# aiforvision/OCTA-autosegmentation

Hardware: AMD Instinct MI355X
Metric: synthetic OCTA samples/sec (graph + 304x304 image + 1216x1216 label triples) (higher is better)
Workload: dtype f64

## Files before the change

### include/octa_hip.h

```cpp
#ifndef OCTA_HIP_H
#define OCTA_HIP_H

#include <stddef.h>
#include <stdint.h>

#ifdef __cplusplus
extern "C" {
#endif

typedef struct octa_ctx octa_ctx;


int octa_abi_version(void);

const char *octa_last_error(void);

int octa_ctx_create(int device, octa_ctx **out);
void octa_ctx_destroy(octa_ctx *ctx);

size_t octa_ctx_scratch_bytes(const octa_ctx *ctx);

int octa_rasterize_2d(octa_ctx *ctx, int B, const double *d_edges, const int64_t *h_edge_off,
                      const uint8_t *d_keep, int no_pixels_x, int no_pixels_y, int mip_axis,
                      double min_radius, double max_radius, uint8_t *d_out, void *stream);
// ... 227 lines not shown

int octa_sim_run_states(octa_sim *sim, const double *h_faz_radius, const double *h_stumps, const uint32_t *h_np_states,
                        const uint32_t *h_py_states, octa_bif_fn bif, void *user, void *stream);
int octa_sim_np_state(octa_sim *sim, int sample, uint32_t *h_state625);

int octa_sim_edge_offsets(octa_sim *sim, int64_t *h_edge_off, int64_t *h_n_art);

int octa_sim_export_edges(octa_sim *sim, double *h_edges);

int octa_sim_export_edges_device(octa_sim *sim, double *d_edges, void *stream);

int octa_sim_trace(octa_sim *sim, int32_t *h_trace);

int octa_sim_stats(octa_sim *sim, int64_t *h_stats);

int octa_sim_spans(octa_sim *sim, int64_t *h_spans);

int octa_sim_timing(octa_sim *sim, double *h_out8);

int octa_sim_service_stats(octa_sim *sim, double *h_out5);

int octa_sim_geometry(int num_cus, int *h_out4);

int octa_sim_is_large(const octa_sim *sim);

int octa_sim_fields(octa_sim *sim, int sample, double *h_oxy, int64_t cap_oxy, int64_t *n_oxy, double *h_co2,
                    int64_t cap_co2, int64_t *n_co2);

int octa_sim_kat_kd_order(octa_ctx *ctx, const double *h_pts, int64_t n, const uint8_t *h_need, int32_t *h_indices);

// ... 5 lines not shown
```

### octa_autosegmentation_amd/_native.py

```python
import contextlib
import ctypes
import os
import random as _random
import threading

import numpy as np

HERE = os.path.dirname(os.path.abspath(__file__))
LIB_PATH = os.environ.get("OCTA_HIP_LIB") or os.path.join(HERE, "liboctahip.so")

_lib = None
_ctxs = {}
_lock = threading.Lock()

c_void_p, c_int, c_double, c_size_t = ctypes.c_void_p, ctypes.c_int, ctypes.c_double, ctypes.c_size_t

SIGNATURES = {
    "octa_abi_version": (c_int, []),
    "octa_last_error": (ctypes.c_char_p, []),
    "octa_ctx_create": (c_int, [c_int, ctypes.POINTER(c_void_p)]),
    "octa_ctx_destroy": (None, [c_void_p]),
    "octa_ctx_scratch_bytes": (c_size_t, [c_void_p]),
    "octa_rasterize_2d": (c_int, [c_void_p, c_int, c_void_p, c_void_p, c_void_p, c_int, c_int, c_int, c_double,
                                  c_double, c_void_p, c_void_p]),
# ... 28 lines not shown
    "octa_sim_destroy": (None, [c_void_p]),
    "octa_sim_run": (c_int, [c_void_p, c_void_p, c_void_p, c_void_p, c_void_p, c_void_p]),
    "octa_sim_run_states": (c_int, [c_void_p, c_void_p, c_void_p, c_void_p, c_void_p, c_void_p, c_void_p, c_void_p]),
    "octa_sim_np_state": (c_int, [c_void_p, c_int, c_void_p]),
    "octa_thinconv_expand": (c_int, [c_void_p, c_void_p, c_void_p, c_void_p, c_void_p, c_int, c_int, c_int, c_int, c_int, c_int, c_int, ctypes.c_float, c_void_p]),
    "octa_thinconv_squeeze": (c_int, [c_void_p, c_void_p, c_void_p, c_void_p, c_void_p, c_int, c_int, c_int, c_int, c_int, c_int, c_int, c_void_p]),
    "octa_lrelu_bwd_bf16": (c_int, [c_void_p, c_void_p, c_void_p, c_void_p, ctypes.c_int64, ctypes.c_float, c_void_p]),
    "octa_thinconv_wgrad_scratch_floats": (ctypes.c_longlong, [c_int, c_int, c_int, c_int]),
    "octa_thinconv_wgrad": (c_int, [c_void_p, c_void_p, c_void_p, c_void_p, c_void_p, c_void_p, c_int, c_int, c_int, c_int, c_int, c_int, c_int, c_int, c_int, c_void_p]),
    "octa_sim_spans": (c_int, [c_void_p, c_void_p]),
    "octa_sim_edge_offsets": (c_int, [c_void_p, c_void_p, c_void_p]),
    "octa_sim_export_edges": (c_int, [c_void_p, c_void_p]),
    "octa_sim_export_edges_device": (c_int, [c_void_p, c_void_p, c_void_p]),
    "octa_sim_trace": (c_int, [c_void_p, c_void_p]),
    "octa_sim_stats": (c_int, [c_void_p, c_void_p]),
    "octa_sim_timing": (c_int, [c_void_p, c_void_p]),
    "octa_sim_service_stats": (c_int, [c_void_p, c_void_p]),
    "octa_sim_geometry": (c_int, [c_int, c_void_p]),
    "octa_sim_is_large": (c_int, [c_void_p]),
    "octa_conv2d_f32_nchw": (c_int, [c_void_p, c_void_p, c_void_p, c_void_p, c_void_p] + [c_int] * 14 + [c_void_p]),
    "octa_convtranspose2x2_f32_nchw": (c_int, [c_void_p, c_void_p, c_void_p, c_void_p, c_int, c_int, c_int, c_int, c_int, c_void_p]),
    "octa_conv2d_f32_dgrad_nchw": (c_int, [c_void_p, c_void_p, c_void_p, c_void_p] + [c_int] * 11 + [c_void_p]),
    "octa_conv2d_f32_wgrad_workspace": (c_int, [c_int] * 10 + [ctypes.POINTER(c_size_t)]),
    "octa_conv2d_f32_wgrad_nchw": (c_int, [c_void_p, c_void_p, c_void_p, c_void_p, c_void_p, c_void_p, c_size_t] + [c_int] * 10 + [c_void_p]),
    "octa_sim_fields": (c_int, [c_void_p, c_int, c_void_p, ctypes.c_int64, c_void_p, c_void_p, ctypes.c_int64, c_void_p]),
    "octa_instnorm_lrelu_nhwc_fwd": (c_int, [c_void_p, c_void_p, c_void_p, c_void_p, c_void_p, c_void_p, c_void_p, c_int, c_int, ctypes.c_int64, ctypes.c_float, ctypes.c_float, c_void_p]),
    "octa_instnorm_lrelu_nhwc_bwd": (c_int, [c_void_p, c_void_p, c_void_p, c_void_p, c_void_p, c_void_p, c_void_p, c_void_p, c_void_p, c_void_p, c_int, c_int, ctypes.c_int64, ctypes.c_float, c_void_p]),
    "octa_head1_nhwc_fwd": (c_int, [c_void_p, c_void_p, c_void_p, ctypes.c_float, ctypes.c_int64, c_int, c_void_p, c_void_p]),
    "octa_head1_nhwc_fwd_b": (c_int, [c_void_p, c_void_p, c_void_p, c_void_p, ctypes.c_int64, c_int, c_void_p, c_void_p]),
    "octa_pack_conv_weights": (c_int, [c_void_p, c_void_p, c_int, c_void_p, c_void_p]),
# ... 153 lines not shown
```

### octa_autosegmentation_amd/csrc/sim.hip

```cpp

#include <chrono>
#include <vector>

#include "common.h"
#include "sim_host.h"
#include <thread>
#include <atomic>
#include <cstdlib>
#include <cstring>

using namespace OCTA_SIMK;

#if OCTA_SIM_LARGE
#define OCTA_SIM_T octa_simL_impl
#define OCTA_SIM_FN(name) octa_simL_##name
#else
#define OCTA_SIM_T octa_simS_impl
#define OCTA_SIM_FN(name) octa_simS_##name
#endif
#define octa_sim_create OCTA_SIM_FN(create)
#define octa_sim_destroy OCTA_SIM_FN(destroy)
#define octa_sim_run OCTA_SIM_FN(run)
#define octa_sim_run_states OCTA_SIM_FN(run_states)
#define octa_sim_np_state OCTA_SIM_FN(np_state)
#define octa_sim_edge_offsets OCTA_SIM_FN(edge_offsets)
#define octa_sim_export_edges OCTA_SIM_FN(export_edges)
#define octa_sim_export_edges_device OCTA_SIM_FN(export_edges_device)
#define octa_sim_trace OCTA_SIM_FN(trace)
#define octa_sim_stats OCTA_SIM_FN(stats)
#define octa_sim_fields OCTA_SIM_FN(fields)
#define octa_sim_service_stats OCTA_SIM_FN(service_stats)
#define octa_sim_geometry OCTA_SIM_FN(geometry)
#define octa_sim_spans OCTA_SIM_FN(spans)
#define octa_sim_timing OCTA_SIM_FN(timing)
#define octa_sim_kat_kd_order OCTA_SIM_FN(kat_kd_order)
struct OCTA_SIM_T;
extern "C" void octa_sim_destroy(OCTA_SIM_T *S);
extern "C" long long octa_sim_next_ticket(void);
extern "C" int *octa_sim_launch_flag(int device);

namespace {

constexpr int SIM_THREADS = SIM_THREADS_PER_WG;
constexpr int SIM_WG_PER_CU = 2;
// ... 1217 lines not shown

extern "C" int octa_sim_stats(OCTA_SIM_T *S, int64_t *h_stats) {
    if (!S || !S->ran || !h_stats) { octa::set_error("octa_sim_stats: run the simulation first"); return -2; }
    for (int s = 0; s < S->B; s++) {
        const SampleScalars &sc = S->h_sc[s];
        int64_t *o = h_stats + 32 * s;
        o[0] = sc.err; o[1] = sc.py_pos; o[2] = sc.murray_steps; o[3] = sc.n_bif; o[4] = sc.respec;
        o[5] = sc.n_nodes[0]; o[6] = sc.n_nodes[1];
        memcpy(&o[7], &sc.faz_radius, 8);
        for (int k = 0; k < 16; k++) o[8 + k] = sc.prof[k];
        for (int k = 0; k < 8; k++) o[24 + k] = sc.kdprof[k];
    }
    return 0;
}

extern "C" int octa_sim_fields(OCTA_SIM_T *S, int sample, double *h_oxy, int64_t cap_oxy, int64_t *n_oxy, double *h_co2,
                               int64_t cap_co2, int64_t *n_co2) {
    if (!S || !S->ran || sample < 0 || sample >= S->B) { octa::set_error("octa_sim_fields: bad arguments"); return -2; }
    OCTA_HIP_CHECK(hipSetDevice(S->ctx->device));
    const SampleScalars &sc = S->h_sc[sample];
    if (n_oxy) *n_oxy = sc.n_oxy;
    if (n_co2) *n_co2 = sc.n_co2;
    if (h_oxy) {
        int64_t n = sc.n_oxy < cap_oxy ? sc.n_oxy : cap_oxy;
        OCTA_HIP_CHECK(hipMemcpy(h_oxy, S->P.oxy + (size_t)sample * OCAP * 3, sizeof(double) * 3 * n, hipMemcpyDeviceToHost));
    }
    if (h_co2) {
        int64_t n = sc.n_co2 < cap_co2 ? sc.n_co2 : cap_co2;
        OCTA_HIP_CHECK(hipMemcpy(h_co2, S->P.co2 + (size_t)sample * CCAP * 3, sizeof(double) * 3 * n, hipMemcpyDeviceToHost));
    }
// ... 69 lines not shown
```

### octa_autosegmentation_amd/csrc/sim_api.cpp

```cpp
#include <cstdlib>
#include <cstring>
#include <new>

#include "common.h"

extern "C" {
struct octa_simS_impl;
struct octa_simL_impl;
#define OCTA_DECL(SFX, T)                                                                                                                       \
    int octa_sim##SFX##_create(octa_ctx *, const octa_sim_config *, int, T **);                                                                 \
    void octa_sim##SFX##_destroy(T *);                                                                                                          \
    int octa_sim##SFX##_run(T *, const uint32_t *, const uint64_t *, octa_bif_fn, void *, void *);                                              \
    int octa_sim##SFX##_run_states(T *, const double *, const double *, const uint32_t *, const uint32_t *, octa_bif_fn, void *, void *);       \
    int octa_sim##SFX##_np_state(T *, int, uint32_t *);                                                                                         \
    int octa_sim##SFX##_edge_offsets(T *, int64_t *, int64_t *);                                                                                \
    int octa_sim##SFX##_export_edges(T *, double *);                                                                                            \
    int octa_sim##SFX##_export_edges_device(T *, double *, void *);                                                                             \
    int octa_sim##SFX##_trace(T *, int32_t *);                                                                                                  \
    int octa_sim##SFX##_stats(T *, int64_t *);                                                                                                  \
    int octa_sim##SFX##_spans(T *, int64_t *);                                                                                                  \
    int octa_sim##SFX##_timing(T *, double *);                                                                                                  \
    int octa_sim##SFX##_service_stats(T *, double *);                                                                                           \
    int octa_sim##SFX##_geometry(int, int *);                                                                                                   \
    int octa_sim##SFX##_fields(T *, int, double *, int64_t, int64_t *, double *, int64_t, int64_t *);
OCTA_DECL(S, octa_simS_impl)
OCTA_DECL(L, octa_simL_impl)
#undef OCTA_DECL
int octa_simS_kat_kd_order(octa_ctx *, const double *, int64_t, const uint8_t *, int32_t *);
}

#include <atomic>
#include <mutex>
static std::atomic<long long> g_sim_launches{0};
extern "C" long long octa_sim_next_ticket(void) { return g_sim_launches.fetch_add(1, std::memory_order_acq_rel) + 1; }
// ... 56 lines not shown
#define NEED(sim, what) if (!(sim)) { octa::set_error(what ": null simulator"); return -2; }
extern "C" int octa_sim_run(octa_sim *sim, const uint32_t *a, const uint64_t *b, octa_bif_fn f, void *u, void *st) {
    NEED(sim, "octa_sim_run") return FWD(octa_simS_run(sim->s, a, b, f, u, st), octa_simL_run(sim->l, a, b, f, u, st));
}
extern "C" int octa_sim_run_states(octa_sim *sim, const double *fz, const double *stp, const uint32_t *a, const uint32_t *b, octa_bif_fn f, void *u, void *st) {
    NEED(sim, "octa_sim_run_states") return FWD(octa_simS_run_states(sim->s, fz, stp, a, b, f, u, st), octa_simL_run_states(sim->l, fz, stp, a, b, f, u, st));
}
extern "C" int octa_sim_np_state(octa_sim *sim, int k, uint32_t *o) { NEED(sim, "octa_sim_np_state") return FWD(octa_simS_np_state(sim->s, k, o), octa_simL_np_state(sim->l, k, o)); }
extern "C" int octa_sim_edge_offsets(octa_sim *sim, int64_t *a, int64_t *b) { NEED(sim, "octa_sim_edge_offsets") return FWD(octa_simS_edge_offsets(sim->s, a, b), octa_simL_edge_offsets(sim->l, a, b)); }
extern "C" int octa_sim_export_edges(octa_sim *sim, double *e) { NEED(sim, "octa_sim_export_edges") return FWD(octa_simS_export_edges(sim->s, e), octa_simL_export_edges(sim->l, e)); }
extern "C" int octa_sim_export_edges_device(octa_sim *sim, double *e, void *st) {
    NEED(sim, "octa_sim_export_edges_device") return FWD(octa_simS_export_edges_device(sim->s, e, st), octa_simL_export_edges_device(sim->l, e, st));
}
extern "C" int octa_sim_trace(octa_sim *sim, int32_t *t) { NEED(sim, "octa_sim_trace") return FWD(octa_simS_trace(sim->s, t), octa_simL_trace(sim->l, t)); }
extern "C" int octa_sim_stats(octa_sim *sim, int64_t *t) { NEED(sim, "octa_sim_stats") return FWD(octa_simS_stats(sim->s, t), octa_simL_stats(sim->l, t)); }
extern "C" int octa_sim_spans(octa_sim *sim, int64_t *t) { NEED(sim, "octa_sim_spans") return FWD(octa_simS_spans(sim->s, t), octa_simL_spans(sim->l, t)); }
extern "C" int octa_sim_timing(octa_sim *sim, double *t) { NEED(sim, "octa_sim_timing") return FWD(octa_simS_timing(sim->s, t), octa_simL_timing(sim->l, t)); }
extern "C" int octa_sim_service_stats(octa_sim *sim, double *t) { NEED(sim, "octa_sim_service_stats") return FWD(octa_simS_service_stats(sim->s, t), octa_simL_service_stats(sim->l, t)); }
extern "C" int octa_sim_fields(octa_sim *sim, int k, double *o, int64_t co, int64_t *no, double *c, int64_t cc, int64_t *nc) {
    NEED(sim, "octa_sim_fields") return FWD(octa_simS_fields(sim->s, k, o, co, no, c, cc, nc), octa_simL_fields(sim->l, k, o, co, no, c, cc, nc));
}
extern "C" int octa_sim_geometry(int num_cus, int *h_out4) { return octa_simS_geometry(num_cus, h_out4); }
extern "C" int octa_sim_kat_kd_order(octa_ctx *ctx, const double *p, int64_t n, const uint8_t *need, int32_t *o) { return octa_simS_kat_kd_order(ctx, p, n, need, o); }
extern "C" int octa_sim_is_large(const octa_sim *sim) { return sim && sim->large ? 1 : 0; }
```

### octa_autosegmentation_amd/csrc/sim_core.h

```cpp
#pragma once
#include <cmath>
#include <cstdint>
#include <cstring>
#include <algorithm>
#include "gpow.h"
#include "glibc_trig.h"

#ifndef OCTA_SIM_LARGE
#define OCTA_SIM_LARGE 0
#endif
#if OCTA_SIM_LARGE
#define OCTA_SIMK octa_simk_large
#else
#define OCTA_SIMK octa_simk
#endif
namespace OCTA_SIMK {

#if OCTA_SIM_LARGE
typedef unsigned int idx_t;
typedef unsigned long long kdw_t;
constexpr int IDX_BITS = 18;
constexpr int GROUP_BITS = 17;
constexpr int NCAP = 1 << 17;
constexpr int OCAP = 1 << 18;
// ... 89 lines not shown
    int py_pos, py_cap;
    int err;
    int new_begin[2], new_end[2];
    int n_groups[2];
    int n_sorted[2];
    int n_grow[2];
    int pass_tag[2];
    int pass_counter;
    long murray_steps;
    long flush_rounds;
    long murray_deferred;
    long n_bif;
    long respec;
    long prof[16];
    long kdprof[8];
    int resume_it, resume_stage;
    int parked, finished;
    long t_begin, t_end;
    int fl_pending[2];
};

struct SimArrays {
    double *npos[2];
    double *nrad[2];
    double *nkap[2];
    int *npar[2], *nch0[2], *nch1[2];
    unsigned char *nnch[2], *nact[2];
    OCTA_HD double *npos_of(int f) const { return f ? npos[1] : npos[0]; }
    OCTA_HD double *nrad_of(int f) const { return f ? nrad[1] : nrad[0]; }
    OCTA_HD double *nkap_of(int f) const { return f ? nkap[1] : nkap[0]; }
// ... 382 lines not shown
            if (s.key[e] < 0) {
                s.fill++; s.used++;
                s.key[e] = key; s.hash[e] = hash;
                if (!OCTA_UNLIKELY(!((long)s.fill * 5 < (long)s.mask * 3))) return;
                pyset_resize(s, s.used > 50000 ? s.used * 2 : s.used * 4);
                return;
            }
            if (s.hash[e] == hash && s.key[e] == key) return;
            e++;
        } while (probes--);
        perturb >>= 5;
        i = (i * 5 + 1 + perturb) & (unsigned long long)s.mask;
    }
}

constexpr int KD_IDX_BITS = IDX_BITS;
constexpr kdw_t KD_IDX_MASK = ((kdw_t)1 << KD_IDX_BITS) - 1u;
constexpr kdw_t KD_QMAX = ((kdw_t)1 << (8 * (int)sizeof(kdw_t) - KD_IDX_BITS)) - 1u;
static_assert(OCAP <= (1 << KD_IDX_BITS), "kd index bits");
struct KdPair {
    kdw_t *kv;
    const double *pts;
    int d;
};
OCTA_HD inline bool kd_less_w(const KdPair &a, kdw_t x, kdw_t y) {
    if (!OCTA_UNLIKELY(!((x ^ y) >> KD_IDX_BITS))) return x < y;
    const unsigned xi = (unsigned)(x & KD_IDX_MASK), yi = (unsigned)(y & KD_IDX_MASK);
    const double fx = a.pts[3 * xi + a.d], fy = a.pts[3 * yi + a.d];
    if (fx == fy) return xi < yi;
    return fx < fy;
// ... 2303 lines not shown
#else
#define OCTA_SUBPROF(sc, slot, t0) do { (void)(t0); } while (0)
#define OCTA_SUBPROF_T0() 0L
#endif

OCTA_HD inline void phase_satisfy_art(const Blk &b, const SimArrays &A, const SimConst &C, const IterParams &P) {
    const double zext = C.sz;
    SampleScalars *sc = A.sc;
    const int nb = sc->new_begin[0], ne = sc->new_end[0];
    const int n_new = ne - nb, n_oxy = sc->n_oxy;
    if (n_new <= 0 || n_oxy <= 0) return;
    const double ek = P.eps_k, ek2 = ek * ek;
    long t0 = OCTA_SUBPROF_T0();
    for (int i = b.tid; i < n_oxy; i += b.nth) A.removed[i] = 0;
    int *ctl = b.coll() + 100;
    if (b.tid == 0) ctl[0] = 0;
    b.sync();
    {
        int *new_ids = A.tmp_int;
        for (int j = b.tid; j < n_new; j += b.nth) new_ids[j] = nb + j;
        b.sync();
        Grid G = grid_build(b, A, A.npos[0], new_ids, n_new, ek);
        for (int o = b.tid; o < n_oxy; o += b.nth) {
            const V3 p = ld3(A.oxy + 3 * o);
            grid_visit(G, p.x, p.y, ek, [&](int j, const V3 &q) {
                if (sqdist(p, q) <= ek2) {
                    int slot = atomic_add_int(&ctl[0], 1);
                    if (slot < PCAP) A.pairs[slot] = ((unsigned)(j - nb) << IDX_BITS) | (unsigned)o;
                    A.removed[o] = 1;
                }
            });
        }
        b.sync();
    }
    OCTA_SUBPROF(sc, 12, t0);
    int n_pairs = ctl[0];
    if (n_pairs > PCAP) { if (b.tid == 0) atomic_or_int(&sc->err, ERR_PAIR_CAP); n_pairs = PCAP; }
    if (n_new > (1 << (32 - IDX_BITS))) { if (b.tid == 0) atomic_or_int(&sc->err, ERR_PAIR_CAP); }
    b.sync();
    if (n_pairs == 0) return;
    kd_build(b, A.oxy, n_oxy, A.kd_idx, A.kd_rank, reinterpret_cast<float *>(A.hashes) , 0.0, zext, sc->kdprof, A.removed, true);
#if OCTA_SIM_DUP & 1
    kd_build(b, A.oxy, n_oxy, A.kd_idx, A.kd_rank, reinterpret_cast<float *>(A.hashes), 0.0, zext, nullptr, A.removed, true);
#endif
    for (int i = b.tid; i < n_pairs; i += b.nth) {
        unsigned pr = A.pairs[i];
        A.pairs[i] = (pr & ~IDX_MASK) | (unsigned)A.kd_rank[pr & IDX_MASK];
    }
    b.sync();
    OCTA_SUBPROF(sc, 11, t0);
    {
        const int n_ven = sc->n_nodes[1];
        int *rem = A.tmp_int;
        int n_rem = 0;
        {
            const int chunk = (n_oxy + b.nth - 1) / b.nth;
            const int i0 = b.tid * chunk < n_oxy ? b.tid * chunk : n_oxy, i1 = (i0 + chunk < n_oxy) ? i0 + chunk : n_oxy;
            int local = 0;
            for (int o = i0; o < i1; o++) local += A.removed[o] ? 1 : 0;
            int ex;
            n_rem = blk_scan(b, local, &ex);
            int run = ex;
            for (int o = i0; o < i1; o++) if (A.removed[o]) rem[run++] = o;
        }
        b.sync();
// ... 8 lines not shown
            V3 qv[VB];
#pragma unroll
            for (int u = 0; u < VB; u++) { const int j = j0 + u * b.nth; qv[u] = ld3(A.npos[1] + 3 * (j < n_ven ? j : n_ven - 1)); }
#pragma unroll
            for (int u = 0; u < VB; u++) {
                if (j0 + u * b.nth >= n_ven) break;
                const V3 q = qv[u];
                grid_visit(G, q.x, q.y, ek, [&](int o, const V3 &p) {
                    if (sqrt(sqdist(q, p)) <= ek) A.ven_near[o] = 1;
                });
            }
        }
        b.sync();
    }
    OCTA_SUBPROF(sc, 12, t0);
    unsigned *keys = reinterpret_cast<unsigned *>(b.user_of<32>());
    int n_pow2 = 1;
    while (n_pow2 < n_pairs) n_pow2 <<= 1;
    for (int i = b.tid; i < n_pow2; i += b.nth) keys[i] = i < n_pairs ? A.pairs[i] : 0xffffffffu;
    b.sync();
    if (n_pairs > 0) blk_sort_u32(b, keys, n_pow2);
    for (int i = b.tid; i < n_pairs; i += b.nth) A.pairs[i] = keys[i];
    b.sync();
    OCTA_SUBPROF(sc, 13, t0);
    bool set_in_lds = false;
#ifdef OCTA_SIM_DEBUG_SAT
    int dbg_n_ins = -1, dbg_mask = -1, dbg_base = -1;
    const int dbg_n_co2_in = sc->n_co2;
#endif
#if defined(__HIP_DEVICE_COMPILE__)
#if defined(OCTA_SIM_PROF_SET)
    long _pt = (long)wall_clock64();
#define PSP(slot) do { if (b.tid == 0) { long _t = (long)wall_clock64(); sc->kdprof[slot] += _t - _pt; _pt = _t; } } while (0)
#else
#define PSP(slot) do { } while (0)
#endif
    constexpr int EMPTY = 0x7fffffff;
    auto replay = [&](int *own, int *in_key, unsigned long long *in_hash, int *dk, unsigned long long *dh, int *ord0, int *ord1,
                      const int s_max) __attribute__((always_inline)) -> int {
        int n_ins = 0;
        for (int p0 = 0; p0 < n_pairs; p0 += b.nth) {
            const int i = p0 + b.tid;
            int o = -1, take = 0;
            unsigned long long hsh = 0;
            if (i < n_pairs) {
                o = (int)A.kd_idx[keys[i] & IDX_MASK];
                take = A.ven_near[o] ? 0 : 1;
                hsh = A.hashes[o];
            }
            int ex;
            const int tot = blk_scan(b, take, &ex);
            if (take) { in_key[n_ins + ex] = o; in_hash[n_ins + ex] = hsh; }
            n_ins += tot;
        }
        b.sync();
        PSP(0);
        for (int i = b.tid; i < n_ins; i += b.nth) own[in_key[i]] = EMPTY;
        b.sync();
        for (int i = b.tid; i < n_ins; i += b.nth) atomic_min_int(&own[in_key[i]], i);
        b.sync();
        int D = 0;
        for (int p0 = 0; p0 < n_ins; p0 += b.nth) {
            const int i = p0 + b.tid;
            const bool first = i < n_ins && own[in_key[i]] == i;
            int ex;
            const int tot = blk_scan(b, first ? 1 : 0, &ex);
            if (first) { dk[D + ex] = in_key[i]; dh[D + ex] = in_hash[i]; }
            D += tot;
        }
        b.sync();
        PSP(1);
        int S = 8, n_prev = 0;
        int *ord = ord0, *ord_next = ord1;
        while (true) {
            const int thr = (3 * (S - 1) + 4) / 5;
            const int upto = D < thr ? D : thr;
            const unsigned long long mask = (unsigned long long)(S - 1);
            for (int p = n_prev + b.tid; p < upto; p += b.nth) ord[p] = p;
            for (int e = b.tid; e < S; e += b.nth) own[e] = EMPTY;
            b.sync();
            for (int p = b.tid; p < upto; p += b.nth) {
                int cur = p;
                unsigned long long hsh = dh[ord[cur]], i = hsh & mask, perturb = hsh;
                int lin = 0, nlin = (i + 9 <= mask) ? 9 : 0;
                auto next = [&] {
                    if (lin < nlin) { lin++; return; }
                    perturb >>= 5;
                    i = (i * 5 + 1 + perturb) & mask;
                    nlin = (i + 9 <= mask) ? 9 : 0; lin = 0;
                };
                while (true) {
                    const int slot = (int)i + lin;
                    const int old = atomic_min_ret_int(&own[slot], cur);
                    if (old == EMPTY) break;
                    if (old > cur) {
                        cur = old;
                        hsh = dh[ord[cur]]; i = hsh & mask; perturb = hsh; lin = 0; nlin = (i + 9 <= mask) ? 9 : 0;
                        while ((int)i + lin != slot) next();
                    }
                    next();
                }
            }
            b.sync();
            if (D < thr) break;
            const int minused = upto > 50000 ? upto * 2 : upto * 4;
            int newS = 8;
            while (newS <= minused) newS <<= 1;
            if (newS > s_max) { if (b.tid == 0) atomic_or_int(&sc->err, ERR_SET_CAP); break; }
            {
                const int lane = b.tid & 63, wv = b.tid >> 6, nw = (b.nth + 63) >> 6;
                const int seg = ((S + nw * 64 - 1) / (nw * 64)) * 64;
                const int s0 = wv * seg < S ? wv * seg : S, s1 = s0 + seg < S ? s0 + seg : S;
                int c = 0;
                for (int e0 = s0; e0 < s1; e0 += 64) c += (int)__popcll(__ballot(e0 + lane < s1 && own[e0 + lane] != EMPTY));
                int ex;
                blk_scan(b, lane == 0 ? c : 0, &ex);
                int at = __builtin_amdgcn_readfirstlane(ex);
                for (int e0 = s0; e0 < s1; e0 += 64) {
                    const int pr = e0 + lane < s1 ? own[e0 + lane] : EMPTY;
                    const unsigned long long m = __ballot(pr != EMPTY);
                    if (pr != EMPTY) ord_next[at + (int)__popcll(m & ((1ull << lane) - 1ull))] = ord[pr];
                    at += (int)__popcll(m);
                }
            }
            b.sync();
            { int *t = ord; ord = ord_next; ord_next = t; }
            n_prev = upto;
            S = newS;
        }
        PSP(2);
        for (int e = b.tid; e < S; e += b.nth) { const int pr = own[e]; own[e] = pr == EMPTY ? -1 : dk[ord[pr]]; }
        b.sync();
        PSP(3);
#ifdef OCTA_SIM_DEBUG_SAT
        dbg_n_ins = n_ins;
#endif
        return S - 1;
    };
    constexpr bool HBM_REPLAY = (size_t)PCAP + OCAP <= (size_t)OCAP + 2 * (size_t)NCANDCAP && (size_t)OCAP * 2 <= (size_t)OCAP * 3
                                && PCAP <= SETCAP && OCAP <= SETCAP;
    const int *t_key = nullptr;
    int mask = -1;
    if (n_pairs <= LSET_PAIRS) {
        constexpr int S_MAX = LSET_CAP / 2;
        int *own = reinterpret_cast<int *>(b.user_of<64>());
        constexpr int OWN_N = OCAP > S_MAX ? OCAP : S_MAX;
        int *in_key = own + OWN_N;
        int *dk = in_key + LSET_PAIRS, *ord0 = dk + LSET_PAIRS, *ord1 = ord0 + LSET_PAIRS;
        unsigned long long *in_hash = reinterpret_cast<unsigned long long *>(ord1 + LSET_PAIRS + ((OWN_N + 4 * LSET_PAIRS) & 1));
        unsigned long long *dh = in_hash + LSET_PAIRS;
        static_assert((size_t)(OWN_N + 4 * LSET_PAIRS + 1) * 4 + (size_t)2 * LSET_PAIRS * 8 <= (size_t)SIM_USER_BYTES, "set replay layout");
        static_assert((size_t)LSET_PAIRS * 4 <= (size_t)OWN_N * 4, "the sorted pairs (start of the table area) end before the insert stream");
        mask = replay(own, in_key, in_hash, dk, dh, ord0, ord1, S_MAX);
        t_key = own;
        set_in_lds = true;
    } else if (HBM_REPLAY && n_pairs <= PCAP) {
        int *own = A.set_key;
        int *in_key = A.tmp_int, *ord0 = A.tmp_int + PCAP;
        unsigned long long *in_hash = A.set_hash;
        unsigned long long *dh = reinterpret_cast<unsigned long long *>(A.tmp_dbl);
        int *dk = reinterpret_cast<int *>(A.tmp_dbl + OCAP), *ord1 = dk + OCAP;
        mask = replay(own, in_key, in_hash, dk, dh, ord0, ord1, SETCAP / 2);
        t_key = own;
        set_in_lds = true;
    }
    if (set_in_lds) {
        const int n_co2_0 = sc->n_co2;
        int base = 0;
        {
            const int per = (mask + 1 + b.nth - 1) / b.nth;
            const int e0 = b.tid * per < mask + 1 ? b.tid * per : mask + 1, e1 = e0 + per < mask + 1 ? e0 + per : mask + 1;
            int cnt = 0;
            for (int e = e0; e < e1; e++) cnt += t_key[e] >= 0 ? 1 : 0;
            int ex2;
            base = blk_scan(b, cnt, &ex2);
            int dst = n_co2_0 + ex2;
            constexpr int RB = 8;
            for (int eb = e0; eb < e1; eb += RB) {
                int k[RB];
                V3 v[RB];
#pragma unroll
                for (int u = 0; u < RB; u++) { k[u] = eb + u < e1 ? t_key[eb + u] : -1; }
#pragma unroll
                for (int u = 0; u < RB; u++) v[u] = ld3(A.oxy + 3 * (k[u] >= 0 ? k[u] : 0));
#pragma unroll
                for (int u = 0; u < RB; u++)
                    if (k[u] >= 0) { if (dst < CCAP) st3(A.co2 + 3 * dst, v[u]); dst++; }
            }
        }
        b.sync();
        PSP(4);
        if (b.tid == 0) {
            int n_co2 = n_co2_0 + base;
            if (n_co2 > CCAP) { sc->err |= ERR_CO2_CAP; n_co2 = CCAP; }
            sc->n_co2 = n_co2;
        }
#ifdef OCTA_SIM_DEBUG_SAT
        dbg_mask = mask; dbg_base = base;
#endif
    }
#undef PSP
#endif
    if (!set_in_lds && b.tid == 0) {
        PySetView S;
        S.hash = A.set_hash; S.key = A.set_key; S.err = &sc->err; S.cap = SETCAP;
        pyset_init(S);
        for (int i = 0; i < n_pairs; i++) {
            int o = (int)A.kd_idx[A.pairs[i] & IDX_MASK];
            if (!A.ven_near[o]) pyset_add(S, o, A.hashes[o]);
        }
        int n_co2 = sc->n_co2;
        for (int e = 0; e <= S.mask; e++)
            if (S.key[e] >= 0) {
                if (n_co2 >= CCAP) { sc->err |= ERR_CO2_CAP; break; }
                int o = S.key[e];
                A.co2[3 * n_co2] = A.oxy[3 * o]; A.co2[3 * n_co2 + 1] = A.oxy[3 * o + 1]; A.co2[3 * n_co2 + 2] = A.oxy[3 * o + 2];
                n_co2++;
            }
        sc->n_co2 = n_co2;
    }
    b.sync();
    OCTA_SUBPROF(sc, 14, t0);
#if defined(OCTA_SIM_DEBUG_SAT) && !defined(OCTA_SIM_ITER_PROF)
    {
        int ex, loc;
        loc = 0; for (int o = b.tid; o < n_oxy; o += b.nth) loc += A.removed[o] ? 1 : 0;
        const int c_rem = blk_scan(b, loc, &ex);
        loc = 0; for (int o = b.tid; o < n_oxy; o += b.nth) loc += (A.removed[o] && A.ven_near[o]) ? 1 : 0;
        const int c_ven = blk_scan(b, loc, &ex);
        unsigned char *mark = reinterpret_cast<unsigned char *>(A.tmp_dbl);
        for (int o = b.tid; o < 2 * n_oxy; o += b.nth) mark[o] = 0;
        b.sync();
        for (int i = b.tid; i < n_pairs; i += b.nth) {
            const int o = (int)A.kd_idx[A.pairs[i] & IDX_MASK];
            mark[o] = 1;
            if (!A.ven_near[o]) mark[n_oxy + o] = 1;
        }
        b.sync();
        loc = 0; for (int o = b.tid; o < n_oxy; o += b.nth) loc += mark[o];
        const int c_pair_all = blk_scan(b, loc, &ex);
        loc = 0; for (int o = b.tid; o < n_oxy; o += b.nth) loc += mark[n_oxy + o];
        const int c_pair_take = blk_scan(b, loc, &ex);
        loc = 0; for (int o = b.tid; o < n_oxy; o += b.nth) loc += (mark[o] != (A.removed[o] ? 1 : 0)) ? 1 : 0;
        const int c_pair_vs_removed = blk_scan(b, loc, &ex);
        int c_slots = -1, c_in_distinct = -1, c_slot_bad = -1;
        if (set_in_lds) {
            const int *t_key = reinterpret_cast<const int *>(b.user());
            const int *in_key = t_key + (OCAP > LSET_CAP / 2 ? OCAP : LSET_CAP / 2);
            loc = 0; for (int e = b.tid; e <= dbg_mask; e += b.nth) loc += t_key[e] >= 0 ? 1 : 0;
            c_slots = blk_scan(b, loc, &ex);
            loc = 0; for (int e = b.tid; e <= dbg_mask; e += b.nth) { const int k = t_key[e]; if (k >= 0 && (k >= n_oxy || !A.removed[k] || A.ven_near[k])) loc++; }
            c_slot_bad = blk_scan(b, loc, &ex);
            for (int o = b.tid; o < n_oxy; o += b.nth) mark[o] = 0;
            b.sync();
            for (int i = b.tid; i < dbg_n_ins; i += b.nth) { const int k = in_key[i]; if (k >= 0 && k < n_oxy) mark[k] = 1; }
            b.sync();
            loc = 0; for (int o = b.tid; o < n_oxy; o += b.nth) loc += mark[o];
            c_in_distinct = blk_scan(b, loc, &ex);
        }
        b.sync();
        if (b.tid == 0 && A.dbg) {
            int *row = A.dbg + 16 * A.dbg_it;
            row[0] = n_new; row[1] = n_oxy; row[2] = n_pairs; row[3] = c_rem; row[4] = c_ven; row[5] = c_pair_all; row[6] = c_pair_take;
            row[7] = c_pair_vs_removed; row[8] = dbg_n_ins; row[9] = dbg_mask; row[10] = dbg_base; row[11] = c_slots; row[12] = c_in_distinct;
            row[13] = c_slot_bad; row[14] = dbg_n_co2_in; row[15] = sc->n_co2;
        }
        b.sync();
    }
#endif
    int keep = compact_points(b, A.oxy, n_oxy, A.removed, A.tmp_dbl);
// ... 34 lines not shown
```

Measured before the change: 1284.

## Skip k-d tree build when set insertion order is independent of kd ranking

Adds a first pass that replays the set insertion using raw point indices sorted by pair key instead of kd ranks, and checks whether the resulting hash-set layout could depend on the ordering within groups. If no order-dependent collisions are detected, the kd_build and rank remap are skipped entirely. Otherwise it falls back to the original kd-ranked path. This adds a verification pass and extra sorting work on the fallback path, and it adds a kd_paths counter API for diagnostics.

```diff
diff --git a/include/octa_hip.h b/include/octa_hip.h
--- a/include/octa_hip.h
+++ b/include/octa_hip.h
@@ -265,6 +265,8 @@
 
 int octa_sim_stats(octa_sim *sim, int64_t *h_stats);
 
+int octa_sim_kd_paths(octa_sim *sim, int64_t *h_paths);
+
 int octa_sim_spans(octa_sim *sim, int64_t *h_spans);
 
 int octa_sim_timing(octa_sim *sim, double *h_out8);
diff --git a/octa_autosegmentation_amd/_native.py b/octa_autosegmentation_amd/_native.py
--- a/octa_autosegmentation_amd/_native.py
+++ b/octa_autosegmentation_amd/_native.py
@@ -66,6 +66,7 @@
     "octa_sim_export_edges_device": (c_int, [c_void_p, c_void_p, c_void_p]),
     "octa_sim_trace": (c_int, [c_void_p, c_void_p]),
     "octa_sim_stats": (c_int, [c_void_p, c_void_p]),
+    "octa_sim_kd_paths": (c_int, [c_void_p, c_void_p]),
     "octa_sim_timing": (c_int, [c_void_p, c_void_p]),
     "octa_sim_service_stats": (c_int, [c_void_p, c_void_p]),
     "octa_sim_geometry": (c_int, [c_int, c_void_p]),
diff --git a/octa_autosegmentation_amd/csrc/sim.hip b/octa_autosegmentation_amd/csrc/sim.hip
--- a/octa_autosegmentation_amd/csrc/sim.hip
+++ b/octa_autosegmentation_amd/csrc/sim.hip
@@ -28,6 +28,7 @@
 #define octa_sim_export_edges_device OCTA_SIM_FN(export_edges_device)
 #define octa_sim_trace OCTA_SIM_FN(trace)
 #define octa_sim_stats OCTA_SIM_FN(stats)
+#define octa_sim_kd_paths OCTA_SIM_FN(kd_paths)
 #define octa_sim_fields OCTA_SIM_FN(fields)
 #define octa_sim_service_stats OCTA_SIM_FN(service_stats)
 #define octa_sim_geometry OCTA_SIM_FN(geometry)
@@ -1275,6 +1276,12 @@
     return 0;
 }
 
+extern "C" int octa_sim_kd_paths(OCTA_SIM_T *S, int64_t *h_paths) {
+    if (!S || !S->ran || !h_paths) { octa::set_error("octa_sim_kd_paths: run the simulation first"); return -2; }
+    for (int s = 0; s < S->B; s++) { h_paths[2 * s] = S->h_sc[s].kd_path[0]; h_paths[2 * s + 1] = S->h_sc[s].kd_path[1]; }
+    return 0;
+}
+
 extern "C" int octa_sim_fields(OCTA_SIM_T *S, int sample, double *h_oxy, int64_t cap_oxy, int64_t *n_oxy, double *h_co2,
                                int64_t cap_co2, int64_t *n_co2) {
     if (!S || !S->ran || sample < 0 || sample >= S->B) { octa::set_error("octa_sim_fields: bad arguments"); return -2; }
diff --git a/octa_autosegmentation_amd/csrc/sim_api.cpp b/octa_autosegmentation_amd/csrc/sim_api.cpp
--- a/octa_autosegmentation_amd/csrc/sim_api.cpp
+++ b/octa_autosegmentation_amd/csrc/sim_api.cpp
@@ -18,6 +18,7 @@
     int octa_sim##SFX##_export_edges_device(T *, double *, void *);                                                                             \
     int octa_sim##SFX##_trace(T *, int32_t *);                                                                                                  \
     int octa_sim##SFX##_stats(T *, int64_t *);                                                                                                  \
+    int octa_sim##SFX##_kd_paths(T *, int64_t *);                                                                                               \
     int octa_sim##SFX##_spans(T *, int64_t *);                                                                                                  \
     int octa_sim##SFX##_timing(T *, double *);                                                                                                  \
     int octa_sim##SFX##_service_stats(T *, double *);                                                                                           \
@@ -104,6 +105,7 @@
 }
 extern "C" int octa_sim_trace(octa_sim *sim, int32_t *t) { NEED(sim, "octa_sim_trace") return FWD(octa_simS_trace(sim->s, t), octa_simL_trace(sim->l, t)); }
 extern "C" int octa_sim_stats(octa_sim *sim, int64_t *t) { NEED(sim, "octa_sim_stats") return FWD(octa_simS_stats(sim->s, t), octa_simL_stats(sim->l, t)); }
+extern "C" int octa_sim_kd_paths(octa_sim *sim, int64_t *t) { NEED(sim, "octa_sim_kd_paths") return FWD(octa_simS_kd_paths(sim->s, t), octa_simL_kd_paths(sim->l, t)); }
 extern "C" int octa_sim_spans(octa_sim *sim, int64_t *t) { NEED(sim, "octa_sim_spans") return FWD(octa_simS_spans(sim->s, t), octa_simL_spans(sim->l, t)); }
 extern "C" int octa_sim_timing(octa_sim *sim, double *t) { NEED(sim, "octa_sim_timing") return FWD(octa_simS_timing(sim->s, t), octa_simL_timing(sim->l, t)); }
 extern "C" int octa_sim_service_stats(octa_sim *sim, double *t) { NEED(sim, "octa_sim_service_stats") return FWD(octa_simS_service_stats(sim->s, t), octa_simL_service_stats(sim->l, t)); }
diff --git a/octa_autosegmentation_amd/csrc/sim_core.h b/octa_autosegmentation_amd/csrc/sim_core.h
--- a/octa_autosegmentation_amd/csrc/sim_core.h
+++ b/octa_autosegmentation_amd/csrc/sim_core.h
@@ -127,6 +127,7 @@
     long respec;
     long prof[16];
     long kdprof[8];
+    int kd_path[2];
     int resume_it, resume_stage;
     int parked, finished;
     long t_begin, t_end;
@@ -539,6 +540,49 @@
     }
 }
 
+OCTA_HD inline bool pyset_order_free(const int *dk, const int *dg, const unsigned long long *hashes, int D, int *own, int *ord0, int *ord1,
+                                     int s_max) {
+    int S = 8, n_prev = 0;
+    int *ord = ord0, *ord_next = ord1;
+    while (true) {
+        const int thr = (3 * (S - 1) + 4) / 5;
+        const int upto = D < thr ? D : thr;
+        const unsigned long long mask = (unsigned long long)(S - 1);
+        for (int p = n_prev; p < upto; p++) ord[p] = p;
+        for (int e = 0; e < S; e++) own[e] = -1;
+        for (int p = 0; p < upto; p++) {
+            const int k = ord[p];
+            const unsigned long long hsh = hashes[dk[k]];
+            unsigned long long perturb = hsh, i = hsh & mask;
+            while (true) {
+                unsigned long long e = i;
+                int probes = (i + 9 <= mask) ? 9 : 0;
+                bool placed = false;
+                do {
+                    const int q = own[e];
+                    if (q < 0) { own[e] = p; placed = true; break; }
+                    if (p >= n_prev && q >= n_prev && dg[q] == dg[k]) return false;
+                    e++;
+                } while (probes--);
+                if (placed) break;
+                perturb >>= 5;
+                i = (i * 5 + 1 + perturb) & mask;
+            }
+        }
+        if (D < thr) return true;
+        if (D > thr && dg[thr - 1] == dg[thr]) return false;
+        const int minused = upto > 50000 ? upto * 2 : upto * 4;
+        int newS = 8;
+        while (newS <= minused) newS <<= 1;
+        if (newS > s_max) return false;
+        int c = 0;
+        for (int e = 0; e < S; e++) if (own[e] >= 0) ord_next[c++] = ord[own[e]];
+        { int *t = ord; ord = ord_next; ord_next = t; }
+        n_prev = upto;
+        S = newS;
+    }
+}
+
 constexpr int KD_IDX_BITS = IDX_BITS;
 constexpr kdw_t KD_IDX_MASK = ((kdw_t)1 << KD_IDX_BITS) - 1u;
 constexpr kdw_t KD_QMAX = ((kdw_t)1 << (8 * (int)sizeof(kdw_t) - KD_IDX_BITS)) - 1u;
@@ -2872,7 +2916,7 @@
     long t0 = OCTA_SUBPROF_T0();
     for (int i = b.tid; i < n_oxy; i += b.nth) A.removed[i] = 0;
     int *ctl = b.coll() + 100;
-    if (b.tid == 0) ctl[0] = 0;
+    if (b.tid == 0) { ctl[0] = 0; ctl[1] = 0; }
     b.sync();
     {
         int *new_ids = A.tmp_int;
@@ -2897,16 +2941,6 @@
     if (n_new > (1 << (32 - IDX_BITS))) { if (b.tid == 0) atomic_or_int(&sc->err, ERR_PAIR_CAP); }
     b.sync();
     if (n_pairs == 0) return;
-    kd_build(b, A.oxy, n_oxy, A.kd_idx, A.kd_rank, reinterpret_cast<float *>(A.hashes) , 0.0, zext, sc->kdprof, A.removed, true);
-#if OCTA_SIM_DUP & 1
-    kd_build(b, A.oxy, n_oxy, A.kd_idx, A.kd_rank, reinterpret_cast<float *>(A.hashes), 0.0, zext, nullptr, A.removed, true);
-#endif
-    for (int i = b.tid; i < n_pairs; i += b.nth) {
-        unsigned pr = A.pairs[i];
-        A.pairs[i] = (pr & ~IDX_MASK) | (unsigned)A.kd_rank[pr & IDX_MASK];
-    }
-    b.sync();
-    OCTA_SUBPROF(sc, 11, t0);
     {
         const int n_ven = sc->n_nodes[1];
         int *rem = A.tmp_int;
@@ -2945,213 +2979,263 @@
         b.sync();
     }
     OCTA_SUBPROF(sc, 12, t0);
-    unsigned *keys = reinterpret_cast<unsigned *>(b.user_of<32>());
-    int n_pow2 = 1;
-    while (n_pow2 < n_pairs) n_pow2 <<= 1;
-    for (int i = b.tid; i < n_pow2; i += b.nth) keys[i] = i < n_pairs ? A.pairs[i] : 0xffffffffu;
-    b.sync();
-    if (n_pairs > 0) blk_sort_u32(b, keys, n_pow2);
-    for (int i = b.tid; i < n_pairs; i += b.nth) A.pairs[i] = keys[i];
-    b.sync();
-    OCTA_SUBPROF(sc, 13, t0);
-    bool set_in_lds = false;
+    bool set_in_lds = false, ranked = false;
 #ifdef OCTA_SIM_DEBUG_SAT
     int dbg_n_ins = -1, dbg_mask = -1, dbg_base = -1;
     const int dbg_n_co2_in = sc->n_co2;
 #endif
+    for (int pass = 0; pass < 2; pass++) {
+        ranked = pass > 0;
+        if (ranked) {
+            kd_build(b, A.oxy, n_oxy, A.kd_idx, A.kd_rank, reinterpret_cast<float *>(A.tmp_dbl), 0.0, zext, sc->kdprof, A.removed, true);
+#if OCTA_SIM_DUP & 1
+            kd_build(b, A.oxy, n_oxy, A.kd_idx, A.kd_rank, reinterpret_cast<float *>(A.tmp_dbl), 0.0, zext, nullptr, A.removed, true);
+#endif
+            for (int i = b.tid; i < n_pairs; i += b.nth) {
+                unsigned pr = A.pairs[i];
+                A.pairs[i] = (pr & ~IDX_MASK) | (unsigned)A.kd_rank[pr & IDX_MASK];
+            }
+            b.sync();
+            OCTA_SUBPROF(sc, 11, t0);
+        }
+        unsigned *keys = reinterpret_cast<unsigned *>(b.user_of<32>());
+        int n_pow2 = 1;
+        while (n_pow2 < n_pairs) n_pow2 <<= 1;
+        for (int i = b.tid; i < n_pow2; i += b.nth) keys[i] = i < n_pairs ? A.pairs[i] : 0xffffffffu;
+        b.sync();
+        if (n_pairs > 0) blk_sort_u32(b, keys, n_pow2);
+        for (int i = b.tid; i < n_pairs; i += b.nth) A.pairs[i] = keys[i];
+        b.sync();
+        OCTA_SUBPROF(sc, 13, t0);
 #if defined(__HIP_DEVICE_COMPILE__)
 #if defined(OCTA_SIM_PROF_SET)
-    long _pt = (long)wall_clock64();
+        long _pt = (long)wall_clock64();
 #define PSP(slot) do { if (b.tid == 0) { long _t = (long)wall_clock64(); sc->kdprof[slot] += _t - _pt; _pt = _t; } } while (0)
 #else
 #define PSP(slot) do { } while (0)
 #endif
-    constexpr int EMPTY = 0x7fffffff;
-    auto replay = [&](int *own, int *in_key, unsigned long long *in_hash, int *dk, unsigned long long *dh, int *ord0, int *ord1,
-                      const int s_max) __attribute__((always_inline)) -> int {
-        int n_ins = 0;
-        for (int p0 = 0; p0 < n_pairs; p0 += b.nth) {
-            const int i = p0 + b.tid;
-            int o = -1, take = 0;
-            unsigned long long hsh = 0;
-            if (i < n_pairs) {
-                o = (int)A.kd_idx[keys[i] & IDX_MASK];
-                take = A.ven_near[o] ? 0 : 1;
-                hsh = A.hashes[o];
-            }
-            int ex;
-            const int tot = blk_scan(b, take, &ex);
-            if (take) { in_key[n_ins + ex] = o; in_hash[n_ins + ex] = hsh; }
-            n_ins += tot;
+        constexpr int EMPTY = 0x7fffffff;
+        auto replay = [&](int *own, int *in_key, unsigned long long *in_hash, int *dk, unsigned long long *dh, int *ord0, int *ord1,
+                          const int s_max) __attribute__((always_inline)) -> int {
+            int n_ins = 0;
+            for (int p0 = 0; p0 < n_pairs; p0 += b.nth) {
+                const int i = p0 + b.tid;
+                int o = -1, take = 0;
+                unsigned long long hsh = 0;
+                if (i < n_pairs) {
+                    o = ranked ? (int)A.kd_idx[keys[i] & IDX_MASK] : (int)(keys[i] & IDX_MASK);
+                    take = A.ven_near[o] ? 0 : 1;
+                    hsh = A.hashes[o];
+                }
+                int ex;
+                const int tot = blk_scan(b, take, &ex);
+                if (take) { in_key[n_ins + ex] = (int)((keys[i] & ~IDX_MASK) | (unsigned)o); in_hash[n_ins + ex] = hsh; }
+                n_ins += tot;
+            }
+            b.sync();
+            PSP(0);
+            for (int i = b.tid; i < n_ins; i += b.nth) own[(unsigned)in_key[i] & IDX_MASK] = EMPTY;
+            b.sync();
+            for (int i = b.tid; i < n_ins; i += b.nth) atomic_min_int(&own[(unsigned)in_key[i] & IDX_MASK], i);
+            b.sync();
+            int D = 0;
+            for (int p0 = 0; p0 < n_ins; p0 += b.nth) {
+                const int i = p0 + b.tid;
+                const bool first = i < n_ins && own[(unsigned)in_key[i] & IDX_MASK] == i;
+                int ex;
+                const int tot = blk_scan(b, first ? 1 : 0, &ex);
+                if (first) { dk[D + ex] = in_key[i]; dh[D + ex] = in_hash[i]; }
+                D += tot;
+            }
+            b.sync();
+            PSP(1);
+            int S = 8, n_prev = 0;
+            int *ord = ord0, *ord_next = ord1;
+            while (true) {
+                const int thr = (3 * (S - 1) + 4) / 5;
+                const int upto = D < thr ? D : thr;
+                const unsigned long long mask = (unsigned long long)(S - 1);
+                for (int p = n_prev + b.tid; p < upto; p += b.nth) ord[p] = p;
+                for (int e = b.tid; e < S; e += b.nth) own[e] = EMPTY;
+                b.sync();
+                for (int p = b.tid; p < upto; p += b.nth) {
+                    int cur = p;
+                    unsigned long long hsh = dh[ord[cur]], i = hsh & mask, perturb = hsh;
+                    int lin = 0, nlin = (i + 9 <= mask) ? 9 : 0;
+                    auto next = [&] {
+                        if (lin < nlin) { lin++; return; }
+                        perturb >>= 5;
+                        i = (i * 5 + 1 + perturb) & mask;
+                        nlin = (i + 9 <= mask) ? 9 : 0; lin = 0;
+                    };
+                    while (true) {
+                        const int slot = (int)i + lin;
+                        const int old = atomic_min_ret_int(&own[slot], cur);
+                        if (old == EMPTY) break;
+                        if (old > cur) {
+                            cur = old;
+                            hsh = dh[ord[cur]]; i = hsh & mask; perturb = hsh; lin = 0; nlin = (i + 9 <= mask) ? 9 : 0;
+                            while ((int)i + lin != slot) next();
+                        }
+                        next();
+                    }
+                }
+                b.sync();
+                if (!ranked) {
+                    for (int p = n_prev + b.tid; p < upto; p += b.nth) {
+                        const unsigned g = (unsigned)dk[p] >> IDX_BITS;
+                        const unsigned long long hsh = dh[p];
+                        unsigned long long i = hsh & mask, perturb = hsh;
+                        int lin = 0, nlin = (i + 9 <= mask) ? 9 : 0;
+                        while (true) {
+                            const int q = own[(int)i + lin];
+                            if (q == p) break;
+                            if (q == EMPTY) { atomic_or_int(&ctl[1], 1); break; }
+                            if (q >= n_prev && ((unsigned)dk[q] >> IDX_BITS) == g) { atomic_or_int(&ctl[1], 1); break; }
+                            if (lin < nlin) { lin++; continue; }
+                            perturb >>= 5;
+                            i = (i * 5 + 1 + perturb) & mask;
+                            nlin = (i + 9 <= mask) ? 9 : 0; lin = 0;
+                        }
+                    }
+                    if (b.tid == 0 && D > thr && ((unsigned)dk[thr - 1] >> IDX_BITS) == ((unsigned)dk[thr] >> IDX_BITS)) atomic_or_int(&ctl[1], 1);
+                    b.sync();
+                    if (ctl[1]) break;
+                }
+                if (D < thr) break;
+                const int minused = upto > 50000 ? upto * 2 : upto * 4;
+                int newS = 8;
+                while (newS <= minused) newS <<= 1;
+                if (newS > s_max) { if (b.tid == 0) atomic_or_int(&sc->err, ERR_SET_CAP); break; }
+                {
+                    const int lane = b.tid & 63, wv = b.tid >> 6, nw = (b.nth + 63) >> 6;
+                    const int seg = ((S + nw * 64 - 1) / (nw * 64)) * 64;
+                    const int s0 = wv * seg < S ? wv * seg : S, s1 = s0 + seg < S ? s0 + seg : S;
+                    int c = 0;
+                    for (int e0 = s0; e0 < s1; e0 += 64) c += (int)__popcll(__ballot(e0 + lane < s1 && own[e0 + lane] != EMPTY));
+                    int ex;
+                    blk_scan(b, lane == 0 ? c : 0, &ex);
+                    int at = __builtin_amdgcn_readfirstlane(ex);
+                    for (int e0 = s0; e0 < s1; e0 += 64) {
+                        const int pr = e0 + lane < s1 ? own[e0 + lane] : EMPTY;
+                        const unsigned long long m = __ballot(pr != EMPTY);
+                        if (pr != EMPTY) ord_next[at + (int)__popcll(m & ((1ull << lane) - 1ull))] = ord[pr];
+                        at += (int)__popcll(m);
+                    }
+                }
+                b.sync();
+                { int *t = ord; ord = ord_next; ord_next = t; }
+                n_prev = upto;
+                S = newS;
+            }
+            PSP(2);
+            for (int e = b.tid; e < S; e += b.nth) { const int pr = own[e]; own[e] = pr == EMPTY ? -1 : (int)((unsigned)dk[ord[pr]] & IDX_MASK); }
+            b.sync();
+            PSP(3);
+#ifdef OCTA_SIM_DEBUG_SAT
+            dbg_n_ins = n_ins;
+#endif
+            return S - 1;
+        };
+        constexpr bool HBM_REPLAY = (size_t)PCAP + OCAP <= (size_t)OCAP + 2 * (size_t)NCANDCAP && (size_t)OCAP * 2 <= (size_t)OCAP * 3
+                                    && PCAP <= SETCAP && OCAP <= SETCAP;
+        const int *t_key = nullptr;
+        int mask = -1;
+        if (n_pairs <= LSET_PAIRS) {
+            constexpr int S_MAX = LSET_CAP / 2;
+            int *own = reinterpret_cast<int *>(b.user_of<64>());
+            constexpr int OWN_N = OCAP > S_MAX ? OCAP : S_MAX;
+            int *in_key = own + OWN_N;
+            int *dk = in_key + LSET_PAIRS, *ord0 = dk + LSET_PAIRS, *ord1 = ord0 + LSET_PAIRS;
+            unsigned long long *in_hash = reinterpret_cast<unsigned long long *>(ord1 + LSET_PAIRS + ((OWN_N + 4 * LSET_PAIRS) & 1));
+            unsigned long long *dh = in_hash + LSET_PAIRS;
+            static_assert((size_t)(OWN_N + 4 * LSET_PAIRS + 1) * 4 + (size_t)2 * LSET_PAIRS * 8 <= (size_t)SIM_USER_BYTES, "set replay layout");
+            static_assert((size_t)LSET_PAIRS * 4 <= (size_t)OWN_N * 4, "the sorted pairs (start of the table area) end before the insert stream");
+            mask = replay(own, in_key, in_hash, dk, dh, ord0, ord1, S_MAX);
+            t_key = own;
+            set_in_lds = true;
+        } else if (HBM_REPLAY && n_pairs <= PCAP) {
+            int *own = A.set_key;
+            int *in_key = A.tmp_int, *ord0 = A.tmp_int + PCAP;
+            unsigned long long *in_hash = A.set_hash;
+            unsigned long long *dh = reinterpret_cast<unsigned long long *>(A.tmp_dbl);
+            int *dk = reinterpret_cast<int *>(A.tmp_dbl + OCAP), *ord1 = dk + OCAP;
+            mask = replay(own, in_key, in_hash, dk, dh, ord0, ord1, SETCAP / 2);
+            t_key = own;
+            set_in_lds = true;
+        }
+        if (set_in_lds && (ranked || !ctl[1])) {
+            const int n_co2_0 = sc->n_co2;
+            int base = 0;
+            {
+                const int per = (mask + 1 + b.nth - 1) / b.nth;
+                const int e0 = b.tid * per < mask + 1 ? b.tid * per : mask + 1, e1 = e0 + per < mask + 1 ? e0 + per : mask + 1;
+                int cnt = 0;
+                for (int e = e0; e < e1; e++) cnt += t_key[e] >= 0 ? 1 : 0;
+                int ex2;
+                base = blk_scan(b, cnt, &ex2);
+                int dst = n_co2_0 + ex2;
+                constexpr int RB = 8;
+                for (int eb = e0; eb < e1; eb += RB) {
+                    int k[RB];
+                    V3 v[RB];
+#pragma unroll
+                    for (int u = 0; u < RB; u++) { k[u] = eb + u < e1 ? t_key[eb + u] : -1; }
+#pragma unroll
+                    for (int u = 0; u < RB; u++) v[u] = ld3(A.oxy + 3 * (k[u] >= 0 ? k[u] : 0));
+#pragma unroll
+                    for (int u = 0; u < RB; u++)
+                        if (k[u] >= 0) { if (dst < CCAP) st3(A.co2 + 3 * dst, v[u]); dst++; }
+                }
+            }
+            b.sync();
+            PSP(4);
+            if (b.tid == 0) {
+                int n_co2 = n_co2_0 + base;
+                if (n_co2 > CCAP) { sc->err |= ERR_CO2_CAP; n_co2 = CCAP; }
+                sc->n_co2 = n_co2;
+            }
+#ifdef OCTA_SIM_DEBUG_SAT
+            dbg_mask = mask; dbg_base = base;
+#endif
+        }
+#undef PSP
+#endif
+        if (!set_in_lds && b.tid == 0) {
+            PySetView S;
+            S.hash = A.set_hash; S.key = A.set_key; S.err = &sc->err; S.cap = SETCAP;
+            pyset_init(S);
+            int *cw = reinterpret_cast<int *>(A.tmp_dbl);
+            static_assert((size_t)SETCAP / 2 <= (size_t)2 * OCAP, "certificate table");
+            int D = 0;
+            for (int i = 0; i < n_pairs; i++) {
+                const unsigned pr = A.pairs[i];
+                const int o = ranked ? (int)A.kd_idx[pr & IDX_MASK] : (int)(pr & IDX_MASK);
+                if (!A.ven_near[o]) {
+                    const int used = S.used;
+                    pyset_add(S, o, A.hashes[o]);
+                    if (!ranked && S.used != used) { cw[D] = o; cw[OCAP + D] = (int)(pr >> IDX_BITS); D++; }
+                }
+            }
+            if (!ranked && !pyset_order_free(cw, cw + OCAP, A.hashes, D, cw + 4 * OCAP, cw + 2 * OCAP, cw + 3 * OCAP, SETCAP / 2)) ctl[1] = 1;
+            if (ranked || !ctl[1]) {
+                int n_co2 = sc->n_co2;
+                for (int e = 0; e <= S.mask; e++)
+                    if (S.key[e] >= 0) {
+                        if (n_co2 >= CCAP) { sc->err |= ERR_CO2_CAP; break; }
+                        int o = S.key[e];
+                        A.co2[3 * n_co2] = A.oxy[3 * o]; A.co2[3 * n_co2 + 1] = A.oxy[3 * o + 1]; A.co2[3 * n_co2 + 2] = A.oxy[3 * o + 2];
+                        n_co2++;
+                    }
+                sc->n_co2 = n_co2;
+            }
         }
         b.sync();
-        PSP(0);
-        for (int i = b.tid; i < n_ins; i += b.nth) own[in_key[i]] = EMPTY;
-        b.sync();
-        for (int i = b.tid; i < n_ins; i += b.nth) atomic_min_int(&own[in_key[i]], i);
-        b.sync();
-        int D = 0;
-        for (int p0 = 0; p0 < n_ins; p0 += b.nth) {
-            const int i = p0 + b.tid;
-            const bool first = i < n_ins && own[in_key[i]] == i;
-            int ex;
-            const int tot = blk_scan(b, first ? 1 : 0, &ex);
-            if (first) { dk[D + ex] = in_key[i]; dh[D + ex] = in_hash[i]; }
-            D += tot;
-        }
-        b.sync();
-        PSP(1);
-        int S = 8, n_prev = 0;
-        int *ord = ord0, *ord_next = ord1;
-        while (true) {
-            const int thr = (3 * (S - 1) + 4) / 5;
-            const int upto = D < thr ? D : thr;
-            const unsigned long long mask = (unsigned long long)(S - 1);
-            for (int p = n_prev + b.tid; p < upto; p += b.nth) ord[p] = p;
-            for (int e = b.tid; e < S; e += b.nth) own[e] = EMPTY;
-            b.sync();
-            for (int p = b.tid; p < upto; p += b.nth) {
-                int cur = p;
-                unsigned long long hsh = dh[ord[cur]], i = hsh & mask, perturb = hsh;
-                int lin = 0, nlin = (i + 9 <= mask) ? 9 : 0;
-                auto next = [&] {
-                    if (lin < nlin) { lin++; return; }
-                    perturb >>= 5;
-                    i = (i * 5 + 1 + perturb) & mask;
-                    nlin = (i + 9 <= mask) ? 9 : 0; lin = 0;
-                };
-                while (true) {
-                    const int slot = (int)i + lin;
-                    const int old = atomic_min_ret_int(&own[slot], cur);
-                    if (old == EMPTY) break;
-                    if (old > cur) {
-                        cur = old;
-                        hsh = dh[ord[cur]]; i = hsh & mask; perturb = hsh; lin = 0; nlin = (i + 9 <= mask) ? 9 : 0;
-                        while ((int)i + lin != slot) next();
-                    }
-                    next();
-                }
-            }
-            b.sync();
-            if (D < thr) break;
-            const int minused = upto > 50000 ? upto * 2 : upto * 4;
-            int newS = 8;
-            while (newS <= minused) newS <<= 1;
-            if (newS > s_max) { if (b.tid == 0) atomic_or_int(&sc->err, ERR_SET_CAP); break; }
-            {
-                const int lane = b.tid & 63, wv = b.tid >> 6, nw = (b.nth + 63) >> 6;
-                const int seg = ((S + nw * 64 - 1) / (nw * 64)) * 64;
-                const int s0 = wv * seg < S ? wv * seg : S, s1 = s0 + seg < S ? s0 + seg : S;
-                int c = 0;
-                for (int e0 = s0; e0 < s1; e0 += 64) c += (int)__popcll(__ballot(e0 + lane < s1 && own[e0 + lane] != EMPTY));
-                int ex;
-                blk_scan(b, lane == 0 ? c : 0, &ex);
-                int at = __builtin_amdgcn_readfirstlane(ex);
-                for (int e0 = s0; e0 < s1; e0 += 64) {
-                    const int pr = e0 + lane < s1 ? own[e0 + lane] : EMPTY;
-                    const unsigned long long m = __ballot(pr != EMPTY);
-                    if (pr != EMPTY) ord_next[at + (int)__popcll(m & ((1ull << lane) - 1ull))] = ord[pr];
-                    at += (int)__popcll(m);
-                }
-            }
-            b.sync();
-            { int *t = ord; ord = ord_next; ord_next = t; }
-            n_prev = upto;
-            S = newS;
-        }
-        PSP(2);
-        for (int e = b.tid; e < S; e += b.nth) { const int pr = own[e]; own[e] = pr == EMPTY ? -1 : dk[ord[pr]]; }
-        b.sync();
-        PSP(3);
-#ifdef OCTA_SIM_DEBUG_SAT
-        dbg_n_ins = n_ins;
-#endif
-        return S - 1;
-    };
-    constexpr bool HBM_REPLAY = (size_t)PCAP + OCAP <= (size_t)OCAP + 2 * (size_t)NCANDCAP && (size_t)OCAP * 2 <= (size_t)OCAP * 3
-                                && PCAP <= SETCAP && OCAP <= SETCAP;
-    const int *t_key = nullptr;
-    int mask = -1;
-    if (n_pairs <= LSET_PAIRS) {
-        constexpr int S_MAX = LSET_CAP / 2;
-        int *own = reinterpret_cast<int *>(b.user_of<64>());
-        constexpr int OWN_N = OCAP > S_MAX ? OCAP : S_MAX;
-        int *in_key = own + OWN_N;
-        int *dk = in_key + LSET_PAIRS, *ord0 = dk + LSET_PAIRS, *ord1 = ord0 + LSET_PAIRS;
-        unsigned long long *in_hash = reinterpret_cast<unsigned long long *>(ord1 + LSET_PAIRS + ((OWN_N + 4 * LSET_PAIRS) & 1));
-        unsigned long long *dh = in_hash + LSET_PAIRS;
-        static_assert((size_t)(OWN_N + 4 * LSET_PAIRS + 1) * 4 + (size_t)2 * LSET_PAIRS * 8 <= (size_t)SIM_USER_BYTES, "set replay layout");
-        static_assert((size_t)LSET_PAIRS * 4 <= (size_t)OWN_N * 4, "the sorted pairs (start of the table area) end before the insert stream");
-        mask = replay(own, in_key, in_hash, dk, dh, ord0, ord1, S_MAX);
-        t_key = own;
-        set_in_lds = true;
-    } else if (HBM_REPLAY && n_pairs <= PCAP) {
-        int *own = A.set_key;
-        int *in_key = A.tmp_int, *ord0 = A.tmp_int + PCAP;
-        unsigned long long *in_hash = A.set_hash;
-        unsigned long long *dh = reinterpret_cast<unsigned long long *>(A.tmp_dbl);
-        int *dk = reinterpret_cast<int *>(A.tmp_dbl + OCAP), *ord1 = dk + OCAP;
-        mask = replay(own, in_key, in_hash, dk, dh, ord0, ord1, SETCAP / 2);
-        t_key = own;
-        set_in_lds = true;
-    }
-    if (set_in_lds) {
-        const int n_co2_0 = sc->n_co2;
-        int base = 0;
-        {
-            const int per = (mask + 1 + b.nth - 1) / b.nth;
-            const int e0 = b.tid * per < mask + 1 ? b.tid * per : mask + 1, e1 = e0 + per < mask + 1 ? e0 + per : mask + 1;
-            int cnt = 0;
-            for (int e = e0; e < e1; e++) cnt += t_key[e] >= 0 ? 1 : 0;
-            int ex2;
-            base = blk_scan(b, cnt, &ex2);
-            int dst = n_co2_0 + ex2;
-            constexpr int RB = 8;
-            for (int eb = e0; eb < e1; eb += RB) {
-                int k[RB];
-                V3 v[RB];
-#pragma unroll
-                for (int u = 0; u < RB; u++) { k[u] = eb + u < e1 ? t_key[eb + u] : -1; }
-#pragma unroll
-                for (int u = 0; u < RB; u++) v[u] = ld3(A.oxy + 3 * (k[u] >= 0 ? k[u] : 0));
-#pragma unroll
-                for (int u = 0; u < RB; u++)
-                    if (k[u] >= 0) { if (dst < CCAP) st3(A.co2 + 3 * dst, v[u]); dst++; }
-            }
-        }
-        b.sync();
-        PSP(4);
-        if (b.tid == 0) {
-            int n_co2 = n_co2_0 + base;
-            if (n_co2 > CCAP) { sc->err |= ERR_CO2_CAP; n_co2 = CCAP; }
-            sc->n_co2 = n_co2;
-        }
-#ifdef OCTA_SIM_DEBUG_SAT
-        dbg_mask = mask; dbg_base = base;
-#endif
-    }
-#undef PSP
-#endif
-    if (!set_in_lds && b.tid == 0) {
-        PySetView S;
-        S.hash = A.set_hash; S.key = A.set_key; S.err = &sc->err; S.cap = SETCAP;
-        pyset_init(S);
-        for (int i = 0; i < n_pairs; i++) {
-            int o = (int)A.kd_idx[A.pairs[i] & IDX_MASK];
-            if (!A.ven_near[o]) pyset_add(S, o, A.hashes[o]);
-        }
-        int n_co2 = sc->n_co2;
-        for (int e = 0; e <= S.mask; e++)
-            if (S.key[e] >= 0) {
-                if (n_co2 >= CCAP) { sc->err |= ERR_CO2_CAP; break; }
-                int o = S.key[e];
-                A.co2[3 * n_co2] = A.oxy[3 * o]; A.co2[3 * n_co2 + 1] = A.oxy[3 * o + 1]; A.co2[3 * n_co2 + 2] = A.oxy[3 * o + 2];
-                n_co2++;
-            }
-        sc->n_co2 = n_co2;
-    }
-    b.sync();
-    OCTA_SUBPROF(sc, 14, t0);
+        OCTA_SUBPROF(sc, 14, t0);
+        if (!ranked && ctl[1]) continue;
+        if (b.tid == 0) sc->kd_path[ranked ? 1 : 0]++;
+        break;
+    }
 #if defined(OCTA_SIM_DEBUG_SAT) && !defined(OCTA_SIM_ITER_PROF)
     {
         int ex, loc;
@@ -3163,7 +3247,7 @@
         for (int o = b.tid; o < 2 * n_oxy; o += b.nth) mark[o] = 0;
         b.sync();
         for (int i = b.tid; i < n_pairs; i += b.nth) {
-            const int o = (int)A.kd_idx[A.pairs[i] & IDX_MASK];
+            const int o = ranked ? (int)A.kd_idx[A.pairs[i] & IDX_MASK] : (int)(A.pairs[i] & IDX_MASK);
             mark[o] = 1;
             if (!A.ven_near[o]) mark[n_oxy + o] = 1;
         }
@@ -3184,7 +3268,7 @@
             c_slot_bad = blk_scan(b, loc, &ex);
             for (int o = b.tid; o < n_oxy; o += b.nth) mark[o] = 0;
             b.sync();
-            for (int i = b.tid; i < dbg_n_ins; i += b.nth) { const int k = in_key[i]; if (k >= 0 && k < n_oxy) mark[k] = 1; }
+            for (int i = b.tid; i < dbg_n_ins; i += b.nth) { const int k = (int)((unsigned)in_key[i] & IDX_MASK); if (k < n_oxy) mark[k] = 1; }
             b.sync();
             loc = 0; for (int o = b.tid; o < n_oxy; o += b.nth) loc += mark[o];
             c_in_distinct = blk_scan(b, loc, &ex);
```

New measurement: 1401, median of 6. 1.09x the previous value.
